# AY-Liu/Image-Editing-Framework

Hardware: AMD Instinct MI355X
Metric: denoising steps/sec (SD1.5 512x512 P2P edit step, UNet batch 4) (higher is better)
Workload: dtype f16x3; 1 GPU; sd15 UNet (859.5M params) P2P AttentionRefine edit step, 2 prompts x CFG = batch 4, 64x64 latents (512x512 px), 50-step DDIM, guidance 7.5, cross 0.8 / self 0.4, per-step null-text unconditional embeddings (P2P_NTI, edit_real.py); one independent edit per GPU; precision mode f16x3: fp32 storage; every contraction on split operands: hi + lo fp16 halves of each fp32 element, Ah Bh + Al Bh + Ah Bl =

## Files before the change

### image-editing-framework_amd/csrc/gemm_x3p.hip

```cpp
#include "ief_common.h"
#include "ief_params.h"
#include "x3_common.h"

#include "x3p_common.h"

template <int BM, int BN, int WAVES_M, int WAVES_N, int NS, int NL, bool CONV>
__global__ __launch_bounds__(64 * (WAVES_M * WAVES_N + NL)) void igemm_x3p_kernel(const IefGemmX3pParams p) {
    constexpr int BK = XP_BK;
    constexpr int NWC = WAVES_M * WAVES_N;
    constexpr int NSW = NL > 0 ? NL : NWC;
    constexpr int PA = BM / 16, PB = BN / 16;
    constexpr int P = 2 * (PA + PB);
    constexpr int G = (P + NSW - 1) / NSW;
    constexpr int WM = BM / WAVES_M, WN = BN / WAVES_N, TM = WM / 16, TN = WN / 16;
    constexpr int SLOT = P * 16 * BK;
    constexpr int DUMP = NS * SLOT;
    static_assert(BM % 16 == 0 && BN % 16 == 0 && WM % 16 == 0 && WN % 16 == 0, "tile");
    static_assert(NS >= 2 && NS <= 4, "ring depth");
    static_assert((NS * SLOT + 512) * 2 <= 160 * 1024, "LDS");
    __shared__ __attribute__((aligned(1024))) half_t smem[NS * SLOT + 512];

    const int tid = threadIdx.x, lane = tid & 63;
    const int wave = __builtin_amdgcn_readfirstlane(tid >> 6);
    const int wr = wave / WAVES_N, wc = wave % WAVES_N;
    const bool stages_ = NL == 0 || wave >= NWC;
    const bool computes = NL == 0 || wave < NWC;
    const int swave = NL > 0 ? wave - NWC : wave;
    const int ntn = (p.N + BN - 1) / BN, ntm = (p.M + BM - 1) / BM;
    const int bid = xcd_remap(blockIdx.x, ntm * ntn);
// ... 23 lines not shown
#pragma unroll
    for (int j = 0; j < G; ++j) {
        const int q = swave + NSW * j;
        exists[j] = stages_ && q < P;
        isA[j] = q < 2 * PA;
        int blk;
        if (isA[j]) { plane[j] = q / PA; blk = q - plane[j] * PA; }
        else { const int q2 = q - 2 * PA; plane[j] = q2 / PB; blk = q2 - plane[j] * PB; }
        ptr[j] = zp; step[j] = 0;
        a_ok[j] = a_live[j] = false; a_y[j] = a_x[j] = a_b[j] = 0; a_m[j] = r1[j] = r2[j] = 0;
        if (!exists[j]) continue;
        if (isA[j]) {
            const int m = m0 + 16 * blk + prow;
            a_ok[j] = m < p.M;
            a_m[j] = (unsigned)m;
            if constexpr (CONV) {
                const int hw = p.Ho * p.Wo;
                const int b = m / hw, rem = m - b * hw;
                const int oy = rem / p.Wo, ox = rem - oy * p.Wo;
                a_b[j] = b;
                a_y[j] = oy * p.stride - (p.pad_hi_only ? 0 : 1);
                a_x[j] = ox * p.stride - (p.pad_hi_only ? 0 : 1);
            } else if (a_ok[j]) {
                ptr[j] = (const char*)p.A + ((long long)plane[j] * p.planeA + (long long)m * p.lda) * 2 + kcb + (long long)kt_lo * (BK * 2);
                step[j] = BK * 2;
            }
        } else {
            const int n = n0 + xp_perm_col<WN>(16 * blk + prow, p.geglu != 0);
            if (n < p.N) {
                ptr[j] = (const char*)p.W + ((long long)plane[j] * p.planeW + (long long)n * p.ldw) * 2 + kcb + (long long)kt_lo * (BK * 2);
                step[j] = BK * 2;
            }
        }
    }

    unsigned stepmask = 0;
#pragma unroll
    for (int j = 0; j < G; ++j) stepmask |= (step[j] != 0 ? 1u : 0u) << j;
    const int Ctot = p.C1 + p.C2;
    const int Hp = p.H >> p.ups, Wp = p.Wd >> p.ups;
    int it_tap = 0, it_c = 0;
    auto set_tap = [&](int tap) {
        if (tap < 9) {
            const int ky = tap / 3, kx = tap - ky * 3;
#pragma unroll
            for (int j = 0; j < G; ++j) {
                if (!(exists[j] && isA[j])) continue;
// ... 8 lines not shown
            for (int j = 0; j < G; ++j) {
                if (!(exists[j] && isA[j])) continue;
                a_live[j] = a_ok[j];
                r1[j] = a_m[j] * (unsigned)p.CE1 * 2u + kcb;
                r2[j] = a_m[j] * (unsigned)p.CE2 * 2u + kcb;
            }
        }
    };
    auto set_src = [&]() {
        const bool tapm = it_tap < 9;
        const int c1 = tapm ? p.C1 : p.CE1;
        const bool first = it_c < c1;
        const char* src = (const char*)(tapm ? (first ? p.A : p.A2) : (first ? p.E1 : p.E2));
        const long long pl = tapm ? (first ? p.planeA : p.planeA2) : (first ? p.planeE1 : p.planeE2);
        const unsigned cc = (unsigned)(first ? it_c : it_c - c1) * 2u;
#pragma unroll
        for (int j = 0; j < G; ++j) {
            if (!(exists[j] && isA[j])) continue;
            ptr[j] = a_live[j] ? src + (long long)plane[j] * pl * 2 + ((first ? r1[j] : r2[j]) + cc) : zp;
            step[j] = a_live[j] ? BK * 2 : 0;
        }
    };

    auto stage_tile = [&](int buf) {
        if (!stages_) return;
        half_t* base = smem + buf * SLOT + swave * (16 * BK);
#pragma unroll
        for (int j = 0; j < G; ++j) {
            half_t* dst = (swave + NSW * j < P) ? base + NSW * j * (16 * BK) : smem + DUMP;
            glds16(ptr[j], dst);
            if constexpr (TN > 5 && !CONV) ptr[j] += ((stepmask >> j) & 1u) ? BK * 2 : 0;
            else ptr[j] += step[j];
        }
        if constexpr (CONV) {
            it_c += BK;
            if (it_tap < 9) {
                if (it_c >= Ctot) { it_c = 0; ++it_tap; set_tap(it_tap); set_src(); }
                else if (it_c == p.C1) set_src();
            } else if (it_c == p.CE1 && p.CE2 > 0) {
                set_src();
            }
        }
    };

    f32x4 acc[TN][TM];
#pragma unroll
    for (int j = 0; j < TN; ++j)
#pragma unroll
        for (int i = 0; i < TM; ++i) acc[j][i] = f32x4{0.f, 0.f, 0.f, 0.f};

    if constexpr (CONV) {
        const int k0 = kt_lo * BK;
        if (k0 < 9 * Ctot) { it_tap = k0 / Ctot; it_c = k0 - it_tap * Ctot; }
        else { it_tap = 9; it_c = k0 - 9 * Ctot; }
        set_tap(it_tap);
// ... 270 lines not shown
    return IEF_OK;
}

extern "C" int ief_gemm_x3p_tile_bm(int tile) {
    switch (tile) {
        case 1: case 2: case 3: case 7: return 128;
        case 4: case 8: case 11: case 12: case 13: return 256;
        case 5: return 64;
        case 6: return 128;
        default: return 0;
    }
}
extern "C" int ief_gemm_x3p_tile_wn(int tile) { return tile == 6 ? 64 : tile == 8 ? 160 : 80; }
extern "C" int ief_gemm_x3p_tile_bn(int tile) {
    switch (tile) {
        case 1: case 2: case 4: case 5: case 7: return 160;
        case 3: case 11: case 12: case 13: return 80;
        case 6: return 64;
        case 8: return 320;
        default: return 0;
    }
}

template <int BM, int BN, int WAVES_M, int WAVES_N, int NS, int NL>
static int launch_x3p(const IefGemmX3pParams& p, hipStream_t st) {
    const int tiles = ((p.M + BM - 1) / BM) * ((p.N + BN - 1) / BN);
    const int splits = p.splits > 1 ? p.splits : 1;
    constexpr int NT = 64 * (WAVES_M * WAVES_N + NL);
    if (p.conv) hipLaunchKernelGGL((igemm_x3p_kernel<BM, BN, WAVES_M, WAVES_N, NS, NL, true>), dim3(tiles, splits), dim3(NT), 0, st, p);
    else hipLaunchKernelGGL((igemm_x3p_kernel<BM, BN, WAVES_M, WAVES_N, NS, NL, false>), dim3(tiles, splits), dim3(NT), 0, st, p);
    IEF_LAUNCH_CHECK();
    return IEF_OK;
}

int ief_conv_halo_x3p_dispatch(const IefGemmX3pParams& p, hipStream_t st);

extern "C" int ief_gemm_x3p(const IefGemmX3pParams* pp, void* stream) {
    if (!pp || !pp->A || !pp->W || !pp->zeros || (!pp->Out && !pp->OutP)) return IEF_EINVAL;
    IefGemmX3pParams p = *pp;
    if (p.M <= 0 || p.N <= 0 || p.K <= 0 || (p.K % XP_BK) || (p.N & 3)) return IEF_ESHAPE;
    if (p.rowvec && p.rows_per_batch <= 0) return IEF_ESHAPE;
    if (p.splits > 1 && (!p.ws || p.splits > 64 || p.geglu || p.rstat_out || p.cstat_out)) return IEF_EINVAL;
    if (!(p.inv_scale > 0.f)) return IEF_EINVAL;
    if ((p.ldw & 7) || (p.planeW & 7) || ((uintptr_t)p.W & 15)) return IEF_EALIGN;
    if (p.Out && ((p.ldo & 3) || ((uintptr_t)p.Out & 15))) return IEF_EALIGN;
    if (p.OutP && ((p.ldp & 3) || (p.planeO & 3) || ((uintptr_t)p.OutP & 7))) return IEF_EALIGN;
    if ((p.bias && ((uintptr_t)p.bias & 15)) || (p.rowvec && ((uintptr_t)p.rowvec & 15)) ||
        (p.residual && (((uintptr_t)p.residual & 15) || (p.ldr & 3)))) return IEF_EALIGN;
    if (p.geglu && ((p.N & 15) || p.residual || p.rowvec)) return IEF_EINVAL;
    if (p.rstat_out && (p.splits > 1 || p.geglu || p.tile == 11 || p.tile == 12 || p.tile == 13 || (p.N % ief_gemm_x3p_tile_wn(p.tile)))) return IEF_EINVAL;
    if (p.rstat_in && (!p.colsum || p.rstat_slots <= 0 || p.rstat_cnt <= 0 || p.rstat_slots * p.rstat_cnt != p.K || p.splits > 1 ||
                       p.conv || !(p.ln_eps > 0.f) || ((uintptr_t)p.colsum & 15))) return IEF_EINVAL;
    if (p.conv) {
        if (p.C1 <= 0 || p.C2 < 0 || (p.C1 % XP_BK) || (p.C2 % XP_BK) || (p.CE1 % XP_BK) || (p.CE2 % XP_BK)) return IEF_ESHAPE;
        if ((p.C2 > 0 && !p.A2) || (p.CE1 > 0 && !p.E1) || (p.CE2 > 0 && !p.E2) || (p.CE2 > 0 && p.CE1 == 0)) return IEF_EINVAL;
        if (p.stride != 1 && p.stride != 2) return IEF_ESHAPE;
        if (p.ups != 0 && p.ups != 1) return IEF_ESHAPE;
        if (p.ups && ((p.H | p.Wd) & 1)) return IEF_ESHAPE;
        if ((p.CE1 + p.CE2) > 0 && (p.stride != 1 || p.ups)) return IEF_ESHAPE;
        const int ktaps = p.tile == 13 ? 4 : 9;
        if (p.K != ktaps * (p.C1 + p.C2) + p.CE1 + p.CE2 || p.batch_images <= 0 || p.M != p.batch_images * p.Ho * p.Wo) return IEF_ESHAPE;
        const long long in_pix = (long long)p.batch_images * (p.H >> p.ups) * (p.Wd >> p.ups);
        const int cmax = p.C1 > p.C2 ? p.C1 : p.C2, emax = p.CE1 > p.CE2 ? p.CE1 : p.CE2;
        if (in_pix * cmax * 2 >= (1ll << 32) || (long long)p.M * emax * 2 >= (1ll << 32)) return IEF_ESHAPE;
        if (((uintptr_t)p.A & 15) || (p.planeA & 7) || (p.A2 && (((uintptr_t)p.A2 & 15) || (p.planeA2 & 7))) ||
            (p.E1 && (((uintptr_t)p.E1 & 15) || (p.planeE1 & 7))) || (p.E2 && (((uintptr_t)p.E2 & 15) || (p.planeE2 & 7)))) return IEF_EALIGN;
    } else {
        if ((p.lda & 7) || (p.planeA & 7) || ((uintptr_t)p.A & 15)) return IEF_EALIGN;
    }
    hipStream_t st = (hipStream_t)stream;
    int rc;
    switch (p.tile) {
        case 2: rc = launch_x3p<128, 160, 4, 2, 4, 4>(p, st); break;
        case 3: rc = launch_x3p<128, 80, 4, 1, 3, 0>(p, st); break;
        case 4: rc = launch_x3p<256, 160, 4, 2, 3, 0>(p, st); break;
        case 5: rc = launch_x3p<64, 160, 2, 2, 4, 0>(p, st); break;
        case 6: rc = launch_x3p<128, 64, 4, 1, 3, 0>(p, st); break;
        case 7: rc = launch_x3p<128, 160, 2, 2, 2, 0>(p, st); break;
        case 8: rc = launch_x3p<256, 320, 4, 2, 2, 0>(p, st); break;
        case 11: case 12: case 13: rc = ief_conv_halo_x3p_dispatch(p, st); break;
        case 1: default: rc = launch_x3p<128, 160, 4, 2, 4, 0>(p, st); break;
    }
    if (rc) return rc;
    if (p.splits > 1) {
        const long long total = (long long)p.M * (p.N / 4);
        int grid = (int)((total + 255) / 256);
        if (grid > 8192) grid = 8192;
        hipLaunchKernelGGL(x3p_reduce_kernel, dim3(grid), dim3(256), 0, st, p);
        IEF_LAUNCH_CHECK();
    }
    return IEF_OK;
}
```

### image-editing-framework_amd/csrc/split_x3.hip

```cpp
#include "ief_common.h"
#include "ief_params.h"

#include "x3_common.h"

__global__ __launch_bounds__(256) void x3_split_weights_kernel(const float* __restrict__ w, half_t* __restrict__ planes, long long n4,
                                                               float s) {
    for (long long i = (long long)blockIdx.x * 256 + threadIdx.x; i < n4; i += (long long)gridDim.x * 256) {
        half4 h, l;
        split4(((const f32x4*)w)[i], s, h, l);
        ((half4*)planes)[i] = h;
        ((half4*)planes)[n4 + i] = l;
    }
}
extern "C" int ief_x3_split_weights(const float* w, void* planes, long long n, float scale, void* stream) {
    if (!w || !planes) return IEF_EINVAL;
    if (n <= 0 || (n & 3) || !(scale > 0.f)) return IEF_ESHAPE;
    if (((uintptr_t)w & 15) || ((uintptr_t)planes & 7)) return IEF_EALIGN;
    long long grid = (n / 4 + 255) / 256;
    if (grid > 16384) grid = 16384;
    hipLaunchKernelGGL(x3_split_weights_kernel, dim3((unsigned)grid), dim3(256), 0, (hipStream_t)stream, w, (half_t*)planes, n / 4, scale);
    IEF_LAUNCH_CHECK();
    return IEF_OK;
}

// ... 8 lines not shown
        const int n = (int)(r % Cout), ph = (int)(r / Cout);
        const int py = ph >> 1, px = ph & 1, sy = tap >> 1, sx = tap & 1;
        const int ky0 = py ? 2 * sy : sy, ky1 = py ? 1 + sy : 2 * sy;
        const int kx0 = px ? 2 * sx : sx, kx1 = px ? 1 + sx : 2 * sx;
        const f32x4* src = (const f32x4*)w + (long long)n * 9 * C4 + c4;
        f32x4 a = src[(ky0 * 3 + kx0) * C4];
        for (int ky = ky0; ky <= ky1; ++ky)
            for (int kx = kx0; kx <= kx1; ++kx)
                if (ky != ky0 || kx != kx0) a = a + src[(ky * 3 + kx) * C4];
        half4 h, l;
        split4(a, s, h, l);
        ((half4*)planes)[i] = h;
        ((half4*)planes)[n4 + i] = l;
    }
}
extern "C" int ief_x3_upsample_phase_weights(const float* w, void* planes, int Cout, int C, float scale, void* stream) {
    if (!w || !planes) return IEF_EINVAL;
    if (Cout <= 0 || C <= 0 || (C & 3) || !(scale > 0.f)) return IEF_ESHAPE;
    if (((uintptr_t)w & 15) || ((uintptr_t)planes & 7)) return IEF_EALIGN;
    long long grid = (16ll * Cout * (C / 4) + 255) / 256;
    if (grid > 16384) grid = 16384;
    hipLaunchKernelGGL(x3_upsample_phase_weights_kernel, dim3((unsigned)grid), dim3(256), 0, (hipStream_t)stream, w, (half_t*)planes, Cout,
                       C / 4, scale);
    IEF_LAUNCH_CHECK();
    return IEF_OK;
}

template <int WM, int WN, int TM, int TN, int KIND, bool TRANSB, bool BPRE>
__global__ __launch_bounds__(64 * WM * WN, (2 * 2 * 16 * (WM * TM + WN * TN) * YLD * 2 > 80 * 1024) ? (WM * WN) / 4 : (WM * WN) / 2)
void igemm_x3_kernel(const IefGemmF32Params p) {
    constexpr bool CONV = KIND >= X3_CONV;
    constexpr bool HASFAST = KIND == X3_LIN || KIND == X3_CONV;
    constexpr int NTH = 64 * WM * WN;
    constexpr int BM = 16 * WM * TM, BN = 16 * WN * TN;
    constexpr int ROWS = BM + BN;
    constexpr int NA = (BM * 8 + NTH - 1) / NTH;
    constexpr int NBC = BPRE ? 2 * BN * 4 : BN * 8;
    constexpr int NB = (NBC + NTH - 1) / NTH;
    constexpr bool A_EXACT = (BM * 8) % NTH == 0, B_EXACT = NBC % NTH == 0;
    static_assert(!(BPRE && TRANSB), "pre-split planes are [N][K]");
    constexpr unsigned OOB = 0xFFFFFFF0u;
    constexpr unsigned OOBF = 0x80000000u;
    __shared__ __attribute__((aligned(16))) half_t smem_y[2 * 2 * ROWS * YLD];
    const int tid = threadIdx.x, lane = tid & 63, wid = tid >> 6;
    const int wm = wid / WN, wn = wid - wm * WN;
    const int lr = lane & 15, lg = lane >> 4;
// ... 1225 lines not shown
```

### image-editing-framework_amd/hip.py

```python
import collections
import ctypes
import os
from ctypes import byref

import torch

from . import cabi

ABI_VERSION = cabi.defines["IEF_ABI_VERSION"]
REPEAT_MAX_JOBS = cabi.defines["IEF_REPEAT_MAX_JOBS"]
_LIB_PATH = os.environ.get("IEF_HIP_LIB") or os.path.join(os.path.dirname(os.path.abspath(__file__)), "libief_hip.so")
_lib = None


class HipExtensionMissing(RuntimeError):
    pass


IefGemmParams = cabi.structs["IefGemmParams"]
IefAttnParams = cabi.structs["IefAttnParams"]
IefCrossParams = cabi.structs["IefCrossParams"]
IefGemmF32Params = cabi.structs["IefGemmF32Params"]
IefAttnF32Params = cabi.structs["IefAttnF32Params"]
IefRepeatJob = cabi.structs["IefRepeatJob"]
# ... 439 lines not shown
    _x3_planes[key] = (weakref.ref(w), w._version, planes)
    weakref.finalize(w, _x3_planes.pop, key, None)
    return planes


def x3_upsample_phase_planes(w, scale=None):
    scale = X3_SCALE_W if scale is None else scale
    key = (w.data_ptr(), tuple(w.shape), float(scale), "phase")
    hit = _x3_planes.get(key)
    if hit is not None and hit[0]() is w and hit[1] == w._version:
        return hit[2]
    if _capturing() or not w.is_contiguous():
        return None
    if w.dim() != 4 or tuple(w.shape[1:3]) != (3, 3) or w.shape[3] % 4:
        raise ValueError("x3_upsample_phase_planes: weight must be [Cout, 3, 3, C] with C a multiple of 4")
    lib = load()
    n, c = w.shape[0], w.shape[3]
    planes = torch.empty(2, 4, n, 4 * c, dtype=torch.float16, device=w.device)
    _check(lib.ief_x3_upsample_phase_weights(w.data_ptr(), planes.data_ptr(), n, c, float(scale), _stream()), "ief_x3_upsample_phase_weights")
    import weakref
    _x3_planes[key] = (weakref.ref(w), w._version, planes)
    weakref.finalize(w, _x3_planes.pop, key, None)
    return planes


def _set_x3(p, sa, sb, w=None) -> str:
    if _F32_CONTRACT == "x3":
        p.x3, p.sa, p.sb = 1, sa, sb
        if w is not None and X3_PRESPLIT and (w.numel() // w.shape[0]) % 8 == 0:
            planes = x3_weight_planes(w, sb)
            if planes is not None:
                p._planes = planes
                p.Wp = planes.data_ptr()
        return "igemm_x3_kernel"
    return "igemm_f32_kernel"


def _is32(t) -> bool:
    return isinstance(t, torch.Tensor) and t.dtype == torch.float32


def _act32(t, name):
    if not (isinstance(t, torch.Tensor) and t.is_cuda and t.dtype == torch.float32):
        raise TypeError(f"{name}: expected an fp32 device tensor (reference-precision mode), got "
                        f"{type(t).__name__ if not isinstance(t, torch.Tensor) else (t.dtype, t.device)}")
    if t.stride(-1) != 1:
# ... 1921 lines not shown
```

### image-editing-framework_amd/planes.py

```python
import os
from ctypes import byref

import torch

from . import hip
from .hip import IefGemmX3pParams, _check, _dev32, _ptr, _shape, _stream, _Timed, _zeros

ACT_SCALE = 1.0
W_SCALE = hip.X3_SCALE_W


class Planes:
    __slots__ = ("t",)

    def __init__(self, t):
        if not (isinstance(t, torch.Tensor) and t.dtype == torch.float16 and t.dim() >= 2 and t.shape[0] == 2 and t.stride(-1) == 1):
            raise TypeError("Planes: expected an fp16 tensor [2, ...] with a contiguous last dimension")
        if not t.is_cuda:
            raise TypeError("Planes: device tensor expected (no CPU path)")
        self.t = t

    @staticmethod
    def empty(*shape, device):
        return Planes(torch.empty(2, *shape, dtype=torch.float16, device=device))
# ... 212 lines not shown
class RowStats:
    __slots__ = ("buf", "slots", "cnt")

    def __init__(self, buf, slots, cnt):
        self.buf, self.slots, self.cnt = buf, slots, cnt


class FoldedLN:
    __slots__ = ("w", "bias", "colsum", "eps")

    def __init__(self, w, bias, gamma, beta, eps):
        wf = (w * gamma[None, :]).contiguous()
        self.w = wf
        b = w @ beta
        self.bias = (b if bias is None else b + bias).contiguous()
        pl = weight_planes(wf)
        self.colsum = ((pl[0].float().sum(1) + pl[1].float().sum(1)) / W_SCALE).contiguous()
        self.eps = eps


LN_FOLD = os.environ.get("IEF_X3P_FOLD_LN", "0") == "1"


def gemm(a, w, bias=None, residual=None, rowvec=None, rows_per_batch=0, out=None, out_planes=None, out_scale=1.0,
         geglu=False, tile=0, splits=0, row_stats=False, ln=None):
    lib = hip.load()
    if not isinstance(a, Planes):
        raise TypeError("planes.gemm: a must be Planes")
    M, K, lda = a.rows_ld("a")
    N = w.shape[0]
    if w.dim() != 2 or w.shape[1] != K:
        raise ValueError(f"planes.gemm: K mismatch {tuple(w.shape)} vs {K}")
    wp = weight_planes(w)
    p = IefGemmX3pParams()
    p.A, p.planeA, p.lda = a.t.data_ptr(), a.plane, lda
    p.W, p.planeW, p.ldw = wp.data_ptr(), wp.stride(0), K
    No = N // 2 if geglu else N
    o32, op = _out_args(p, M, No, out, out_planes, a.device, a.shape[:-1])
    p.M, p.N, p.K = M, N, K
    p.out_scale, p.inv_scale = out_scale, 1.0 / (ACT_SCALE * W_SCALE)
    p.geglu, p.zeros = 1 if geglu else 0, _zeros(a.device)
    if tile:
        p.tile, p.splits = tile, max(1, splits)
    else:
        key = f"gemm|{M}|{N}|{K}" + ("|g" if geglu else "")
        if AUTOTUNE and key not in _plan_table() and not hip._capturing() and hip._prof is None:
            _autotune(key, candidate_plans(M, N, K, geglu=geglu),
                      lambda t, sp, wi: gemm(a, wi, bias=bias, residual=residual, rowvec=rowvec, rows_per_batch=rows_per_batch, out=out,
                                             out_planes=out_planes, out_scale=out_scale, geglu=geglu, tile=t, splits=sp), w)
        p.tile, p.splits = pick_plan(M, N, K, variant="|g" if geglu else "")
    if geglu or row_stats or ln is not None:
        p.splits = 1
    rs = None
    if row_stats:
        wn = lib.ief_gemm_x3p_tile_wn(p.tile)
        if N % wn:
            raise ValueError("planes.gemm: row statistics need N to be a multiple of the tile's wave width")
        rs = RowStats(torch.empty(M, N // wn, 2, dtype=torch.float32, device=a.device), N // wn, wn)
        p.rstat_out = rs.buf.data_ptr()
    if ln is not None:
        st, colsum, eps = ln
        if st.buf.shape[0] != M or st.slots * st.cnt != K or _dev32(colsum, "colsum").numel() != N:
            raise ValueError("planes.gemm: ln statistics / colsum do not match this launch")
        p.rstat_in, p.rstat_slots, p.rstat_cnt, p.colsum, p.ln_eps = st.buf.data_ptr(), st.slots, st.cnt, colsum.data_ptr(), eps
    ws = hip._fill_epilogue(p, hip._rows_ld32, "planes.gemm", M, N, a.device, bias, rowvec, rows_per_batch, residual, p.splits)
    nbytes = 4.0 * (M * K + N * K + M * No * ((1 if o32 is not None else 0) + (1 if op is not None else 0)) + (M * N if residual is not None else 0))
    kn = f"igemm_x3p_kernel<false> t{p.tile}" + (f" {M}x{N}x{K} s{p.splits}" if hip.PROF_SHAPES else "")
    bm, bn = _TILES[p.tile]
    hip.note_staged(kn, 4.0 * K * (bm + bn) * -(-M // bm) * -(-N // bn))
    with _Timed(kn, 2.0 * M * N * K, nbytes):
        _check(lib.ief_gemm_x3p(byref(p), _stream()), "ief_gemm_x3p")
    r = _ret(o32, op)
    if row_stats:
        return (r + (rs,)) if isinstance(r, tuple) else (r, rs)
    return r


def conv3x3(x, w, bias=None, x2=None, stride=1, upsample=False, rowvec=None, residual=None, out=None, out_planes=None,
            extra=None, pad_hi_only=False, tile=0, splits=0):
    lib = hip.load()
    if not isinstance(x, Planes) or (x2 is not None and not isinstance(x2, Planes)):
        raise TypeError("planes.conv3x3: x / x2 must be Planes")
    if not x.is_contiguous() or (x2 is not None and not x2.is_contiguous()) or not w.is_contiguous():
        raise ValueError("planes.conv3x3: x, x2, w must be contiguous")
    e1, e2 = (None, None) if extra is None else extra
    for e in (e1, e2):
        if e is not None and (not isinstance(e, Planes) or not e.is_contiguous()):
            raise ValueError("planes.conv3x3: extra sources must be contiguous NHWC Planes at the output resolution")
    if residual is not None and not hip._act32(residual, "residual").is_contiguous():
        raise ValueError("planes.conv3x3: residual must be contiguous fp32 [B, Ho, Wo, Cout]")
# ... 270 lines not shown
```

### image-editing-framework_amd/unet.py

```python
import math
import os
from typing import Dict, Optional

import torch
from torch import nn

from . import hip, planes
from .config import UNetConfig


FOLD_LN = os.environ.get("IEF_FOLD_LN", "1") == "1"
KV_ONE_GEMM = os.environ.get("IEF_KV_ONE_GEMM", "1") == "1"


def _fold_ln(w16, bias32, gamma, beta):
    wf = w16.float()
    wp = (wf * gamma[None, :]).half().contiguous()
    b = wf @ beta
    if bias32 is not None:
        b = b + bias32
    return wp, b.contiguous(), wp.float().sum(1).contiguous()


class UNetOutput(dict):
# ... 177 lines not shown
                if plan.second_sources(B, self) is not None:
                    raise RuntimeError(f"{self.layer_name}: the Union plan's two key segments exist on the planes attention of the "
                                       "f16x3 mode only")
            o = hip.attn_flash(q, k, v, self.heads, self.scale, q_src=qs, k_src=ks, v_src=vs)
        else:
            q = hip.gemm(x, self.to_q.weight) if ln is None else hip.gemm(x, self.ln_w, bias=self.ln_b, ln=ln)
            kv = self.context_kv(encoder_hidden_states)
            args = plan.cross_edit(B, self) if plan is not None else {}
            if self.map_out is not None:
                hip.attn_probs(q, kv[..., :C], self.heads, self.scale, out=self.map_out)
            o = hip.attn_cross_p2p(q, kv[..., :C], kv[..., C:], self.heads, self.scale, **args)
        if plan is not None:
            plan.layer_done(self)
        lin = self.to_out[0]
        if want_stats:
            return hip.gemm(o, lin.weight, bias=lin.bias, residual=residual, row_stats=True)
        return lin(o, residual=residual)


    def fold_layernorm_x3p(self, norm):
        w = self.w_qkv if self.w_qkv is not None else self.to_q.weight
        self.ln3 = planes.FoldedLN(w, None, norm.weight, norm.bias, norm.eps)

    def forward_x3p(self, xp, ctx, residual, ln_stats=None, want_stats=False, cfg_rows=None):
        B, N, C = xp.shape
        if cfg_rows is not None:
            if cfg_rows.rows != B:
                raise ValueError("forward_x3p: cfg_rows was built for another batch")
            B = cfg_rows.n
        self.last_tokens = N
        plan = self._plan
        w_in, b_in, ln = (self.w_qkv if ctx is None else self.to_q.weight), None, None
        if ln_stats is not None:
            w_in, b_in, ln = self.ln3.w, self.ln3.bias, (ln_stats, self.ln3.colsum, self.ln3.eps)
        if ctx is None:
            qs = ks = vs = None
            if plan is not None:
                qs, ks, vs = plan.self_sources(B, N, self)
            if cfg_rows is not None and (qs is not None or ks is not None or vs is not None
                                         or (plan is not None and plan.mask_launches(B, N, self) is not None)
                                         or (plan is not None and plan.kind == "masactrl_mask_auto"
                                             and (self._exec_index // 2) in plan.masa_layers)):
                raise RuntimeError(f"{self.layer_name}: the control plan acts on a self-attention that runs in the shared prefix of a "
                                   "CFG step (ControlPlan.controls_first_self must say so)")
            if planes.FLASH_PLANES and self.dim_head in planes.FLASH_PLANES_DIMS:
                qkv = planes.gemm(xp, w_in, bias=b_in, ln=ln, out=False, out_planes=True)
                k2 = plan.second_sources(B, self) if plan is not None else None
# ... 18 lines not shown
                qkv = planes.gemm(xp, w_in, bias=b_in, ln=ln)
                if plan is not None and (plan.mask_launches(B, N, self) is not None or plan.auto_launch(B, N, self) is not None):
                    raise RuntimeError(f"mask-guided MasaCtrl was lowered onto a layer of head dim {self.dim_head} that has no "
                                       "planes attention")
                if plan is not None and plan.second_sources(B, self) is not None:
                    raise RuntimeError(f"MasaCtrl Union was lowered onto a layer of head dim {self.dim_head} that has no planes "
                                       "attention")
                o = hip.attn_flash(qkv[..., :C], qkv[..., C:2 * C], qkv[..., 2 * C:], self.heads, self.scale, q_src=qs, k_src=ks,
                                   v_src=vs, out_planes=True)
        else:
            q = planes.gemm(xp, w_in, bias=b_in, ln=ln)
            kv = self.context_kv(ctx)
            args = plan.cross_edit(B, self) if plan is not None else {}
            if self.map_out is not None:
                hip.attn_probs(q, kv[..., :C], self.heads, self.scale, out=self.map_out)
            if plan is not None:
                plan.cross_mass(B, N, self, q, kv[..., :C])
            o = hip.attn_cross_p2p(q, kv[..., :C], kv[..., C:], self.heads, self.scale, out_planes=True, q_src=cfg_rows, **args)
        if plan is not None:
            plan.layer_done(self)
        lin = self.to_out[0]
        if want_stats:
            return planes.gemm(o, lin.weight, bias=lin.bias, residual=residual, out=True, out_planes=True, row_stats=True)
        return planes.gemm(o, lin.weight, bias=lin.bias, residual=residual)


class GEGLU(nn.Module):

    def __init__(self, sd, prefix, dev):
        super().__init__()
        w, b = sd[prefix + ".proj.weight"], sd[prefix + ".proj.bias"]
        half = w.shape[0] // 2
        il = lambda t: torch.stack([t[:half].reshape(half // 8, 8, *t.shape[1:]),
                                    t[half:].reshape(half // 8, 8, *t.shape[1:])], 1).reshape(t.shape)
        self.proj = Linear(_f16(il(w), dev), _f32(il(b), dev))
        self.proj.interleaved = True

    def fold_layernorm(self, norm):
        self.ln_w, self.ln_b, self.ln_c1 = _fold_ln(self.proj.weight, self.proj.bias, norm.weight, norm.bias)
        self.ln_eps = norm.eps

    def forward(self, x, ln_stats=None):
        if ln_stats is not None:
            return hip.gemm(x, self.ln_w, bias=self.ln_b, geglu=True, ln=(ln_stats, self.ln_c1, self.ln_eps))
        return hip.gemm(x, self.proj.weight, bias=self.proj.bias, geglu=True)

# ... 56 lines not shown
        f0 = self.ff.net[0].proj
        self.ff.net[0].ln3 = planes.FoldedLN(f0.weight, f0.bias, self.norm3.weight, self.norm3.bias, self.norm3.eps)

    def foldable_x3p(self):
        if not (planes.LN_FOLD and self.attn1.is_native() and self.attn2.is_native()):
            return False
        if getattr(self.attn1, "ln3", None) is None:
            if hip._capturing():
                return False
            self.fold_layernorm_x3p()
        return True

    def forward_x3p_folded(self, h, hp, st, ctx, last, want_stats):
        h, hp, st = self.attn1.forward_x3p(hp, None, residual=h, ln_stats=st, want_stats=True)
        h, hp, st = self.attn2.forward_x3p(hp, ctx, residual=h, ln_stats=st, want_stats=True)
        f0, lin = self.ff.net[0], self.ff.net[2]
        g = planes.gemm(hp, f0.ln3.w, bias=f0.ln3.bias, geglu=True, out=False, out_planes=True, ln=(st, f0.ln3.colsum, f0.ln3.eps))
        if last:
            return planes.gemm(g, lin.weight, bias=lin.bias, residual=h, out=False, out_planes=True)
        if want_stats:
            return planes.gemm(g, lin.weight, bias=lin.bias, residual=h, out=True, out_planes=True, row_stats=True)
        return planes.gemm(g, lin.weight, bias=lin.bias, residual=h)

    def forward_x3p(self, h, ctx, last, cfg_rows=None, carry=()):
        if cfg_rows is not None:
            h = self.attn1.forward_x3p(planes.layernorm(h, self.norm1.weight, self.norm1.bias, self.norm1.eps), None, residual=h,
                                       cfg_rows=cfg_rows)
            n2 = planes.layernorm(h, self.norm2.weight, self.norm2.bias, self.norm2.eps)
            rep = hip.repeat_batch(h, *carry)
            h, carry = (rep[0], tuple(rep[1:])) if carry else (rep, ())
            h = self.attn2.forward_x3p(n2, ctx, residual=h, cfg_rows=cfg_rows)
        else:
            h = self._attend_x3p(self.attn1, self.norm1, h, None)
            h = self._attend_x3p(self.attn2, self.norm2, h, ctx)
        n3 = planes.layernorm(h, self.norm3.weight, self.norm3.bias, self.norm3.eps)
        f0, lin = self.ff.net[0].proj, self.ff.net[2]
        g = planes.gemm(n3, f0.weight, bias=f0.bias, geglu=True, out=False, out_planes=True)
        if last:
            r = planes.gemm(g, lin.weight, bias=lin.bias, residual=h, out=False, out_planes=True)
        else:
            r = planes.gemm(g, lin.weight, bias=lin.bias, residual=h)
        return (r, carry) if cfg_rows is not None else r


class Transformer2DModel(nn.Module):
    def __init__(self, sd, prefix, dim, heads, cross_dim, groups, dev, name, depth=1):
        super().__init__()
        self.norm = GroupNorm(_f32(sd[prefix + ".norm.weight"], dev), _f32(sd[prefix + ".norm.bias"], dev), groups, 1e-6)
        c1 = lambda n: Conv2d(_f16(sd[f"{prefix}.{n}.weight"].reshape(dim, dim), dev), _f32(sd[f"{prefix}.{n}.bias"], dev), 1)
        self.proj_in, self.proj_out = c1("proj_in"), c1("proj_out")
        self.transformer_blocks = nn.ModuleList(
            [BasicTransformerBlock(sd, f"{prefix}.transformer_blocks.{k}", dim, heads, cross_dim, dev,
                                   name if k == 0 else f"{name}.b{k}") for k in range(depth)])

    def forward(self, x, encoder_hidden_states=None, cstat=None, col_stats=False):
        B, H, W, C = x.shape
        if all(blk.foldable() for blk in self.transformer_blocks):
            h, st = hip.gemm(self.norm(x, cstat=cstat), self.proj_in.weight, bias=self.proj_in.bias, row_stats=True)
            h = h.reshape(B, H * W, C)
            last = len(self.transformer_blocks) - 1
            for k, blk in enumerate(self.transformer_blocks):
                if k < last:
                    h, st = blk(h, encoder_hidden_states, ln_stats=st, want_stats=True)
                else:
                    h = blk(h, encoder_hidden_states, ln_stats=st)
            return self.proj_out(h.reshape(B, H, W, C), residual=x, col_stats=col_stats)
        h = self.proj_in(self.norm(x, cstat=cstat)).reshape(B, H * W, C)
        for blk in self.transformer_blocks:
            h = blk(h, encoder_hidden_states)
        return self.proj_out(h.reshape(B, H, W, C), residual=x, col_stats=col_stats)


    def forward_x3p(self, x, encoder_hidden_states=None, want_planes=False, cfg_rows=None, carry=()):
        B, H, W, C = x.shape
        n = self.norm
        hn = planes.groupnorm(x, n.weight, n.bias, n.num_groups, n.eps, silu=False)
        last = len(self.transformer_blocks) - 1
        if cfg_rows is not None:
            h = planes.gemm(hn.reshape(B, H * W, C), self.proj_in.weight, bias=self.proj_in.bias)
            for k, blk in enumerate(self.transformer_blocks):
                if k == 0:
                    h, rep = blk.forward_x3p(h, encoder_hidden_states, last=(k == last), cfg_rows=cfg_rows, carry=(x,) + tuple(carry))
                    x, carry = rep[0], rep[1:]
                    B = x.shape[0]
                else:
                    h = blk.forward_x3p(h, encoder_hidden_states, last=(k == last))
        elif all(blk.foldable_x3p() for blk in self.transformer_blocks):
            h, hp, st = planes.gemm(hn.reshape(B, H * W, C), self.proj_in.weight, bias=self.proj_in.bias, out=True, out_planes=True,
                                    row_stats=True)
            for k, blk in enumerate(self.transformer_blocks):
                r = blk.forward_x3p_folded(h, hp, st, encoder_hidden_states, last=(k == last), want_stats=(k < last))
                if k < last:
                    h, hp, st = r
                else:
                    h = r
        else:
            h = planes.gemm(hn.reshape(B, H * W, C), self.proj_in.weight, bias=self.proj_in.bias)
            for k, blk in enumerate(self.transformer_blocks):
                h = blk.forward_x3p(h, encoder_hidden_states, last=(k == last))
        r = planes.gemm(h, self.proj_out.weight, bias=self.proj_out.bias, residual=x.reshape(B, H * W, C), out=True,
                        out_planes=want_planes)
        if want_planes:
            r = r[0].reshape(B, H, W, C), r[1].reshape(B, H, W, C)
        else:
            r = r.reshape(B, H, W, C), None
        return r + (tuple(carry),) if cfg_rows is not None else r


class ResnetBlock2D(nn.Module):

    def __init__(self, sd, prefix, cin, cout, groups, eps, dev, temb_slot):
        super().__init__()
        self.in_channels, self.out_channels = cin, cout
        self.norm1 = GroupNorm(_f32(sd[prefix + ".norm1.weight"], dev), _f32(sd[prefix + ".norm1.bias"], dev), groups, eps)
        self.norm2 = GroupNorm(_f32(sd[prefix + ".norm2.weight"], dev), _f32(sd[prefix + ".norm2.bias"], dev), groups, eps)
        pack = lambda w: _f16(w.permute(0, 2, 3, 1), dev)
        self.conv1 = Conv2d(pack(sd[prefix + ".conv1.weight"]), _f32(sd[prefix + ".conv1.bias"], dev), 3)
        self.time_emb_proj = Linear(_f16(sd[prefix + ".time_emb_proj.weight"], dev), _f32(sd[prefix + ".time_emb_proj.bias"], dev))
        self.nonlinearity = SiLU()
        self.dropout = Dropout()
        self.upsample = self.downsample = None
        self.skip_time_act = False
        self.time_embedding_norm = "default"
        self.output_scale_factor = 1.0
# ... 463 lines not shown
```

### include/ief_hip.h

```cpp
#ifndef IEF_HIP_H
#define IEF_HIP_H
#include <stdint.h>

#ifdef __HIPCC__
typedef _Float16 ief_half;
#else
typedef uint16_t ief_half;
#endif

#ifdef __cplusplus
extern "C" {
#endif

#define IEF_ABI_VERSION 4
int ief_abi_version(void);
const char* ief_target_arch(void);
int ief_struct_size(int which);

typedef struct IefGemmParams {
    const ief_half* A;
    const ief_half* A2;
    const ief_half* W;
    ief_half* Out;
    const float* bias;
// ... 224 lines not shown
    const ief_half* W;  long long planeW;
    float* Out;
    ief_half* OutP; long long planeO;
    const float* bias;
    const float* rowvec;
    const float* residual;
    int M, N, K;
    int lda, ldw, ldo, ldp, ldr;
    int conv, H, Wd, C1, C2, Ho, Wo, stride, ups, batch_images, pad_hi_only, CE1, CE2;
    int rows_per_batch;
    float out_scale;
    float inv_scale;
    int tile;
    int splits;
    float* ws;
    int geglu;
    const void* zeros;
    float* rstat_out;
    float* cstat_out;
    const float* rstat_in;
    const float* colsum;
    int rstat_slots, rstat_cnt;
    float ln_eps;
} IefGemmX3pParams;
int ief_gemm_x3p(const IefGemmX3pParams* p, void* stream);
int ief_x3_upsample_phase_weights(const float* w, void* planes, int Cout, int C, float scale, void* stream);
int ief_gemm_x3p_tile_bm(int tile);
int ief_gemm_x3p_tile_bn(int tile);
int ief_gemm_x3p_tile_wn(int tile);
int ief_x3_split_act(const float* x, ief_half* planes, long long plane, long long rows, int C, int ldx, int ldp, float scale,
                     void* stream);

int ief_groupnorm_bwd_f32(const float* x, const float* x2, int C1, int C2, const float* dy, const float* add, float* dx, float* dx2,
                          const float* gamma, const float* beta, int B, int HW, int groups, float eps, int silu, void* stream);
int ief_layernorm_bwd_f32(const float* x, const float* dy, const float* add, float* dx, const float* gamma, long long rows, int C,
                          float eps, void* stream);
int ief_geglu_il_bwd_f32(const float* pre, const float* dy, float* dpre, long long rows, int Ch, void* stream);
int ief_zero_insert2x_f32(const float* in, float* out, int B, int H, int W, int C, void* stream);
int ief_pool2x2_sum_f32(const float* in, float* out, int B, int H, int W, int C, void* stream);
int ief_conv_out_bwd_f32w(const float* d_eps, const float* w, float* dh, int B, int C, int H, int W, int Cout, void* stream);
int ief_softmax_bwd_rows_f32(const float* P, float* dP, long long rows, int L, float scale, void* stream);
int ief_transpose_batched_f32(const float* in, float* out, int R, int N, int L, void* stream);
int ief_map_loss_rows_blocks(long long rows);
int ief_map_loss_rows_f32(const float* P, const float* ref, float* dP, float* loss, long long rows, int L, float gcoef,
                          float loss_coef, void* stream);
int ief_nti_adam_f32g(float* param, float* m, float* v, const float* grad, const float* stats, const float* hyper, int* step, int n,
                      void* stream);

// ... 82 lines not shown
```

### profiles/make_step_breakdown.py

```python
import csv
import json
import sys


def family(n):
    if n.startswith("igemm_x3p_kernel"):
        return "conv (implicit GEMM on planes)" if n.split("(")[0].rstrip(">").endswith("true") else "linear (igemm_x3p)"
    if n.startswith("conv3x3_halo_x3p"):
        return "conv (halo on planes)"
    if n.startswith("attn_flash"):
        return "self-attention (flash)"
    if n.startswith("attn_cross_p2p"):
        return "cross-attention (fused edit)"
    if "gn3_" in n or "groupnorm" in n:
        return "GroupNorm"
    if "layernorm" in n:
        return "LayerNorm"
    if "reduce" in n:
        return "split-K reducer"
    return "other"


def main():
    rows = list(csv.DictReader(open(sys.argv[1])))
    rows.sort(key=lambda r: int(r["Start_Timestamp"]))
    marks = [i for i, r in enumerate(rows) if "cfg_ddim" in r["Kernel_Name"]]
    a, b = marks[len(marks) // 2] + 1, marks[len(marks) // 2 + 1] + 1
    step = rows[a:b]
    out = {"_what": "one captured step of the headline command (f16x3, SD1.5 512x512, batch 4) from profiles' kernel trace: launches and "
                    "kernel time per family", "launches": len(step)}
# ... 20 lines not shown
```

Measured before the change: 80.43 steps/s.

## Fold FF output linear into proj_out via K-concatenated GEMM

```diff
diff --git a/image-editing-framework_amd/csrc/gemm_x3p.hip b/image-editing-framework_amd/csrc/gemm_x3p.hip
--- a/image-editing-framework_amd/csrc/gemm_x3p.hip
+++ b/image-editing-framework_amd/csrc/gemm_x3p.hip
@@ -4,7 +4,7 @@
 
 #include "x3p_common.h"
 
-template <int BM, int BN, int WAVES_M, int WAVES_N, int NS, int NL, bool CONV>
+template <int BM, int BN, int WAVES_M, int WAVES_N, int NS, int NL, bool CONV, bool KCAT = false>
 __global__ __launch_bounds__(64 * (WAVES_M * WAVES_N + NL)) void igemm_x3p_kernel(const IefGemmX3pParams p) {
     constexpr int BK = XP_BK;
     constexpr int NWC = WAVES_M * WAVES_N;
@@ -74,7 +74,14 @@
                 a_y[j] = oy * p.stride - (p.pad_hi_only ? 0 : 1);
                 a_x[j] = ox * p.stride - (p.pad_hi_only ? 0 : 1);
             } else if (a_ok[j]) {
-                ptr[j] = (const char*)p.A + ((long long)plane[j] * p.planeA + (long long)m * p.lda) * 2 + kcb + (long long)kt_lo * (BK * 2);
+                if constexpr (KCAT) {
+                    const int k1t = p.K1 / BK;
+                    ptr[j] = kt_lo < k1t
+                        ? (const char*)p.A + ((long long)plane[j] * p.planeA + (long long)m * p.lda) * 2 + kcb + (long long)kt_lo * (BK * 2)
+                        : (const char*)p.A2 + ((long long)plane[j] * p.planeA2 + (long long)m * p.lda2) * 2 + kcb + (long long)(kt_lo - k1t) * (BK * 2);
+                } else {
+                    ptr[j] = (const char*)p.A + ((long long)plane[j] * p.planeA + (long long)m * p.lda) * 2 + kcb + (long long)kt_lo * (BK * 2);
+                }
                 step[j] = BK * 2;
             }
         } else {
@@ -129,6 +136,7 @@
         }
     };
 
+    int st_k = kt_lo;
     auto stage_tile = [&](int buf) {
         if (!stages_) return;
         half_t* base = smem + buf * SLOT + swave * (16 * BK);
@@ -138,6 +146,14 @@
             glds16(ptr[j], dst);
             if constexpr (TN > 5 && !CONV) ptr[j] += ((stepmask >> j) & 1u) ? BK * 2 : 0;
             else ptr[j] += step[j];
+        }
+        if constexpr (KCAT) {
+            if (++st_k == p.K1 / BK) {
+#pragma unroll
+                for (int j = 0; j < G; ++j)
+                    if (exists[j] && isA[j] && a_ok[j])
+                        ptr[j] = (const char*)p.A2 + ((long long)plane[j] * p.planeA2 + (long long)a_m[j] * p.lda2) * 2 + kcb;
+            }
         }
         if constexpr (CONV) {
             it_c += BK;
@@ -454,13 +470,17 @@
     }
 }
 
-template <int BM, int BN, int WAVES_M, int WAVES_N, int NS, int NL>
+template <int BM, int BN, int WAVES_M, int WAVES_N, int NS, int NL, bool HAS_KCAT = false>
 static int launch_x3p(const IefGemmX3pParams& p, hipStream_t st) {
     const int tiles = ((p.M + BM - 1) / BM) * ((p.N + BN - 1) / BN);
     const int splits = p.splits > 1 ? p.splits : 1;
     constexpr int NT = 64 * (WAVES_M * WAVES_N + NL);
     if (p.conv) hipLaunchKernelGGL((igemm_x3p_kernel<BM, BN, WAVES_M, WAVES_N, NS, NL, true>), dim3(tiles, splits), dim3(NT), 0, st, p);
-    else hipLaunchKernelGGL((igemm_x3p_kernel<BM, BN, WAVES_M, WAVES_N, NS, NL, false>), dim3(tiles, splits), dim3(NT), 0, st, p);
+    else if (p.K1 > 0) {
+        if constexpr (HAS_KCAT)
+            hipLaunchKernelGGL((igemm_x3p_kernel<BM, BN, WAVES_M, WAVES_N, NS, NL, false, true>), dim3(tiles, splits), dim3(NT), 0, st, p);
+        else return IEF_EINVAL;
+    } else hipLaunchKernelGGL((igemm_x3p_kernel<BM, BN, WAVES_M, WAVES_N, NS, NL, false>), dim3(tiles, splits), dim3(NT), 0, st, p);
     IEF_LAUNCH_CHECK();
     return IEF_OK;
 }
@@ -483,6 +503,12 @@
     if (p.rstat_out && (p.splits > 1 || p.geglu || p.tile == 11 || p.tile == 12 || p.tile == 13 || (p.N % ief_gemm_x3p_tile_wn(p.tile)))) return IEF_EINVAL;
     if (p.rstat_in && (!p.colsum || p.rstat_slots <= 0 || p.rstat_cnt <= 0 || p.rstat_slots * p.rstat_cnt != p.K || p.splits > 1 ||
                        p.conv || !(p.ln_eps > 0.f) || ((uintptr_t)p.colsum & 15))) return IEF_EINVAL;
+    if (p.K1 != 0) {
+        if (p.conv || p.geglu || p.rstat_in || !p.A2) return IEF_EINVAL;
+        if (p.tile != 1 && p.tile != 3 && p.tile != 4 && p.tile != 6) return IEF_EINVAL;
+        if (p.K1 < 0 || p.K1 >= p.K || (p.K1 % XP_BK) || ((p.K - p.K1) % XP_BK)) return IEF_ESHAPE;
+        if ((p.lda2 & 7) || (p.planeA2 & 7) || ((uintptr_t)p.A2 & 15)) return IEF_EALIGN;
+    }
     if (p.conv) {
         if (p.C1 <= 0 || p.C2 < 0 || (p.C1 % XP_BK) || (p.C2 % XP_BK) || (p.CE1 % XP_BK) || (p.CE2 % XP_BK)) return IEF_ESHAPE;
         if ((p.C2 > 0 && !p.A2) || (p.CE1 > 0 && !p.E1) || (p.CE2 > 0 && !p.E2) || (p.CE2 > 0 && p.CE1 == 0)) return IEF_EINVAL;
@@ -504,14 +530,14 @@
     int rc;
     switch (p.tile) {
         case 2: rc = launch_x3p<128, 160, 4, 2, 4, 4>(p, st); break;
-        case 3: rc = launch_x3p<128, 80, 4, 1, 3, 0>(p, st); break;
-        case 4: rc = launch_x3p<256, 160, 4, 2, 3, 0>(p, st); break;
+        case 3: rc = launch_x3p<128, 80, 4, 1, 3, 0, true>(p, st); break;
+        case 4: rc = launch_x3p<256, 160, 4, 2, 3, 0, true>(p, st); break;
         case 5: rc = launch_x3p<64, 160, 2, 2, 4, 0>(p, st); break;
-        case 6: rc = launch_x3p<128, 64, 4, 1, 3, 0>(p, st); break;
+        case 6: rc = launch_x3p<128, 64, 4, 1, 3, 0, true>(p, st); break;
         case 7: rc = launch_x3p<128, 160, 2, 2, 2, 0>(p, st); break;
         case 8: rc = launch_x3p<256, 320, 4, 2, 2, 0>(p, st); break;
         case 11: case 12: case 13: rc = ief_conv_halo_x3p_dispatch(p, st); break;
-        case 1: default: rc = launch_x3p<128, 160, 4, 2, 4, 0>(p, st); break;
+        case 1: default: rc = launch_x3p<128, 160, 4, 2, 4, 0, true>(p, st); break;
     }
     if (rc) return rc;
     if (p.splits > 1) {
diff --git a/image-editing-framework_amd/csrc/split_x3.hip b/image-editing-framework_amd/csrc/split_x3.hip
--- a/image-editing-framework_amd/csrc/split_x3.hip
+++ b/image-editing-framework_amd/csrc/split_x3.hip
@@ -54,6 +54,41 @@
     if (grid > 16384) grid = 16384;
     hipLaunchKernelGGL(x3_upsample_phase_weights_kernel, dim3((unsigned)grid), dim3(256), 0, (hipStream_t)stream, w, (half_t*)planes, Cout,
                        C / 4, scale);
+    IEF_LAUNCH_CHECK();
+    return IEF_OK;
+}
+
+__global__ __launch_bounds__(256) void x3_fold_linear_pair_kernel(const float* __restrict__ wp, const float* __restrict__ w2,
+                                                                  const float* __restrict__ b2, const float* __restrict__ bp,
+                                                                  float* __restrict__ wcat, float* __restrict__ bcat, int C, int K) {
+    const int cols = K + C + 1;
+    const long long total = (long long)C * cols;
+    for (long long i = (long long)blockIdx.x * 256 + threadIdx.x; i < total; i += (long long)gridDim.x * 256) {
+        const int r = (int)(i / cols), c = (int)(i - (long long)r * cols);
+        const float* wr = wp + (long long)r * C;
+        if (c < K) {
+            double a = 0.0;
+            for (int j = 0; j < C; ++j) a += (double)wr[j] * (double)w2[(long long)j * K + c];
+            wcat[(long long)r * (K + C) + c] = (float)a;
+        } else if (c < K + C) {
+            wcat[(long long)r * (K + C) + c] = wr[c - K];
+        } else {
+            double a = 0.0;
+            if (b2)
+                for (int j = 0; j < C; ++j) a += (double)wr[j] * (double)b2[j];
+            if (bp) a += (double)bp[r];
+            bcat[r] = (float)a;
+        }
+    }
+}
+extern "C" int ief_x3_fold_linear_pair(const float* wp, const float* w2, const float* b2, const float* bp, float* wcat, float* bcat,
+                                       int C, int K, void* stream) {
+    if (!wp || !w2 || !wcat || !bcat) return IEF_EINVAL;
+    if (C <= 0 || K <= 0) return IEF_ESHAPE;
+    long long grid = ((long long)C * (K + C + 1) + 255) / 256;
+    if (grid > 16384) grid = 16384;
+    hipLaunchKernelGGL(x3_fold_linear_pair_kernel, dim3((unsigned)grid), dim3(256), 0, (hipStream_t)stream, wp, w2, b2, bp, wcat, bcat, C,
+                       K);
     IEF_LAUNCH_CHECK();
     return IEF_OK;
 }
diff --git a/image-editing-framework_amd/hip.py b/image-editing-framework_amd/hip.py
--- a/image-editing-framework_amd/hip.py
+++ b/image-editing-framework_amd/hip.py
@@ -485,6 +485,44 @@
     _x3_planes[key] = (weakref.ref(w), w._version, planes)
     weakref.finalize(w, _x3_planes.pop, key, None)
     return planes
+
+
+def fold_linear_pair_ref(wp, w2, b2=None, bp=None):
+    wp64, w264 = wp.double(), w2.double()
+    if wp64.dim() != 2 or wp64.shape[0] != wp64.shape[1] or w264.dim() != 2 or w264.shape[0] != wp64.shape[0]:
+        raise ValueError("fold_linear_pair: wp must be [C, C] and w2 [C, K]")
+    b = torch.zeros(wp64.shape[0], dtype=torch.float64, device=wp.device)
+    if b2 is not None:
+        b = wp64 @ b2.double()
+    if bp is not None:
+        b = b + bp.double()
+    return torch.cat([wp64 @ w264, wp64], 1), b
+
+
+def x3_fold_linear_pair(wp, w2, b2=None, bp=None):
+    key = (wp.data_ptr(), tuple(wp.shape), w2.data_ptr(), tuple(w2.shape), "fold")
+    srcs = (wp, w2, b2, bp)
+    hit = _x3_planes.get(key)
+    if hit is not None and all((r is None and t is None) or (r is not None and r() is t and v == t._version)
+                               for t, (r, v) in zip(srcs, hit[0])):
+        return hit[2]
+    if _capturing():
+        return None
+    if wp.dim() != 2 or wp.shape[0] != wp.shape[1] or w2.dim() != 2 or w2.shape[0] != wp.shape[0]:
+        raise ValueError("x3_fold_linear_pair: wp must be [C, C] and w2 [C, K]")
+    C, K = w2.shape
+    for t, nm in ((wp, "wp"), (w2, "w2"), (b2, "b2"), (bp, "bp")):
+        if t is not None and (not _dev32(t, nm).is_contiguous() or (t.dim() == 1 and t.numel() != C)):
+            raise ValueError(f"x3_fold_linear_pair: {nm} must be contiguous fp32 ([C] for a bias)")
+    lib = load()
+    wcat = torch.empty(C, K + C, dtype=torch.float32, device=wp.device)
+    bcat = torch.empty(C, dtype=torch.float32, device=wp.device)
+    _check(lib.ief_x3_fold_linear_pair(wp.data_ptr(), w2.data_ptr(), _ptr(b2), _ptr(bp), wcat.data_ptr(), bcat.data_ptr(), C, K,
+                                       _stream()), "ief_x3_fold_linear_pair")
+    import weakref
+    _x3_planes[key] = (tuple((None, 0) if t is None else (weakref.ref(t), t._version) for t in srcs), 0, (wcat, bcat))
+    weakref.finalize(wp, _x3_planes.pop, key, None)
+    return wcat, bcat
 
 
 def _set_x3(p, sa, sb, w=None) -> str:
diff --git a/image-editing-framework_amd/planes.py b/image-editing-framework_amd/planes.py
--- a/image-editing-framework_amd/planes.py
+++ b/image-editing-framework_amd/planes.py
@@ -258,18 +258,37 @@
 LN_FOLD = os.environ.get("IEF_X3P_FOLD_LN", "0") == "1"
 
 
+KCAT_TILES = (1, 3, 4, 6)
+_KCAT_NEAREST = {2: 1, 5: 1, 7: 1, 8: 4}
+
+
+FOLD_TAIL = os.environ.get("IEF_X3P_FOLD_TAIL", "1") == "1"
+
+
 def gemm(a, w, bias=None, residual=None, rowvec=None, rows_per_batch=0, out=None, out_planes=None, out_scale=1.0,
-         geglu=False, tile=0, splits=0, row_stats=False, ln=None):
+         geglu=False, tile=0, splits=0, row_stats=False, ln=None, a2=None):
     lib = hip.load()
     if not isinstance(a, Planes):
         raise TypeError("planes.gemm: a must be Planes")
     M, K, lda = a.rows_ld("a")
+    K1 = 0
+    if a2 is not None:
+        if not isinstance(a2, Planes):
+            raise TypeError("planes.gemm: a2 must be Planes")
+        if geglu or ln is not None:
+            raise ValueError("planes.gemm: a K-concatenated launch takes no geglu and no folded LayerNorm")
+        M2, K2, lda2 = a2.rows_ld("a2")
+        if M2 != M:
+            raise ValueError(f"planes.gemm: a2 has {M2} rows, a has {M}")
+        K1, K = K, K + K2
     N = w.shape[0]
     if w.dim() != 2 or w.shape[1] != K:
         raise ValueError(f"planes.gemm: K mismatch {tuple(w.shape)} vs {K}")
     wp = weight_planes(w)
     p = IefGemmX3pParams()
     p.A, p.planeA, p.lda = a.t.data_ptr(), a.plane, lda
+    if a2 is not None:
+        p.A2, p.planeA2, p.lda2, p.K1 = a2.t.data_ptr(), a2.plane, lda2, K1
     p.W, p.planeW, p.ldw = wp.data_ptr(), wp.stride(0), K
     No = N // 2 if geglu else N
     o32, op = _out_args(p, M, No, out, out_planes, a.device, a.shape[:-1])
@@ -281,10 +300,13 @@
     else:
         key = f"gemm|{M}|{N}|{K}" + ("|g" if geglu else "")
         if AUTOTUNE and key not in _plan_table() and not hip._capturing() and hip._prof is None:
-            _autotune(key, candidate_plans(M, N, K, geglu=geglu),
+            cands = candidate_plans(M, N, K, geglu=geglu)
+            _autotune(key, [c for c in cands if a2 is None or c[0] in KCAT_TILES],
                       lambda t, sp, wi: gemm(a, wi, bias=bias, residual=residual, rowvec=rowvec, rows_per_batch=rows_per_batch, out=out,
-                                             out_planes=out_planes, out_scale=out_scale, geglu=geglu, tile=t, splits=sp), w)
+                                             out_planes=out_planes, out_scale=out_scale, geglu=geglu, tile=t, splits=sp, a2=a2), w)
         p.tile, p.splits = pick_plan(M, N, K, variant="|g" if geglu else "")
+        if a2 is not None:
+            p.tile = _KCAT_NEAREST.get(p.tile, p.tile)
     if geglu or row_stats or ln is not None:
         p.splits = 1
     rs = None
@@ -301,7 +323,7 @@
         p.rstat_in, p.rstat_slots, p.rstat_cnt, p.colsum, p.ln_eps = st.buf.data_ptr(), st.slots, st.cnt, colsum.data_ptr(), eps
     ws = hip._fill_epilogue(p, hip._rows_ld32, "planes.gemm", M, N, a.device, bias, rowvec, rows_per_batch, residual, p.splits)
     nbytes = 4.0 * (M * K + N * K + M * No * ((1 if o32 is not None else 0) + (1 if op is not None else 0)) + (M * N if residual is not None else 0))
-    kn = f"igemm_x3p_kernel<false> t{p.tile}" + (f" {M}x{N}x{K} s{p.splits}" if hip.PROF_SHAPES else "")
+    kn = f"igemm_x3p_kernel<false>{' kcat' if a2 is not None else ''} t{p.tile}" + (f" {M}x{N}x{K} s{p.splits}" if hip.PROF_SHAPES else "")
     bm, bn = _TILES[p.tile]
     hip.note_staged(kn, 4.0 * K * (bm + bn) * -(-M // bm) * -(-N // bn))
     with _Timed(kn, 2.0 * M * N * K, nbytes):
diff --git a/image-editing-framework_amd/unet.py b/image-editing-framework_amd/unet.py
--- a/image-editing-framework_amd/unet.py
+++ b/image-editing-framework_amd/unet.py
@@ -223,7 +223,7 @@
         w = self.w_qkv if self.w_qkv is not None else self.to_q.weight
         self.ln3 = planes.FoldedLN(w, None, norm.weight, norm.bias, norm.eps)
 
-    def forward_x3p(self, xp, ctx, residual, ln_stats=None, want_stats=False, cfg_rows=None):
+    def forward_x3p(self, xp, ctx, residual, ln_stats=None, want_stats=False, cfg_rows=None, want_planes=False):
         B, N, C = xp.shape
         if cfg_rows is not None:
             if cfg_rows.rows != B:
@@ -288,6 +288,8 @@
         lin = self.to_out[0]
         if want_stats:
             return planes.gemm(o, lin.weight, bias=lin.bias, residual=residual, out=True, out_planes=True, row_stats=True)
+        if want_planes:
+            return planes.gemm(o, lin.weight, bias=lin.bias, residual=residual, out=True, out_planes=True)
         return planes.gemm(o, lin.weight, bias=lin.bias, residual=residual)
 
 
@@ -390,21 +392,30 @@
             return planes.gemm(g, lin.weight, bias=lin.bias, residual=h, out=True, out_planes=True, row_stats=True)
         return planes.gemm(g, lin.weight, bias=lin.bias, residual=h)
 
-    def forward_x3p(self, h, ctx, last, cfg_rows=None, carry=()):
+    def forward_x3p(self, h, ctx, last, cfg_rows=None, carry=(), fold_tail=False):
         if cfg_rows is not None:
             h = self.attn1.forward_x3p(planes.layernorm(h, self.norm1.weight, self.norm1.bias, self.norm1.eps), None, residual=h,
                                        cfg_rows=cfg_rows)
             n2 = planes.layernorm(h, self.norm2.weight, self.norm2.bias, self.norm2.eps)
             rep = hip.repeat_batch(h, *carry)
             h, carry = (rep[0], tuple(rep[1:])) if carry else (rep, ())
-            h = self.attn2.forward_x3p(n2, ctx, residual=h, cfg_rows=cfg_rows)
+            h = self.attn2.forward_x3p(n2, ctx, residual=h, cfg_rows=cfg_rows, want_planes=fold_tail)
         else:
             h = self._attend_x3p(self.attn1, self.norm1, h, None)
-            h = self._attend_x3p(self.attn2, self.norm2, h, ctx)
+            if fold_tail:
+                h = self.attn2.forward_x3p(planes.layernorm(h, self.norm2.weight, self.norm2.bias, self.norm2.eps), ctx, residual=h,
+                                           want_planes=True)
+            else:
+                h = self._attend_x3p(self.attn2, self.norm2, h, ctx)
+        hp = None
+        if fold_tail:
+            h, hp = h
         n3 = planes.layernorm(h, self.norm3.weight, self.norm3.bias, self.norm3.eps)
         f0, lin = self.ff.net[0].proj, self.ff.net[2]
         g = planes.gemm(n3, f0.weight, bias=f0.bias, geglu=True, out=False, out_planes=True)
-        if last:
+        if fold_tail:
+            r = (g, hp)
+        elif last:
             r = planes.gemm(g, lin.weight, bias=lin.bias, residual=h, out=False, out_planes=True)
         else:
             r = planes.gemm(g, lin.weight, bias=lin.bias, residual=h)
@@ -439,20 +450,30 @@
         return self.proj_out(h.reshape(B, H, W, C), residual=x, col_stats=col_stats)
 
 
+    def tail_fold(self):
+        blk = self.transformer_blocks[-1]
+        if not planes.FOLD_TAIL or planes.LN_FOLD or not blk.attn2.is_native():
+            return None
+        lin = blk.ff.net[2]
+        return hip.x3_fold_linear_pair(self.proj_out.weight, lin.weight, lin.bias, self.proj_out.bias)
+
     def forward_x3p(self, x, encoder_hidden_states=None, want_planes=False, cfg_rows=None, carry=()):
         B, H, W, C = x.shape
         n = self.norm
         hn = planes.groupnorm(x, n.weight, n.bias, n.num_groups, n.eps, silu=False)
         last = len(self.transformer_blocks) - 1
+        fold = self.tail_fold()
         if cfg_rows is not None:
             h = planes.gemm(hn.reshape(B, H * W, C), self.proj_in.weight, bias=self.proj_in.bias)
             for k, blk in enumerate(self.transformer_blocks):
+                ft = fold is not None and k == last
                 if k == 0:
-                    h, rep = blk.forward_x3p(h, encoder_hidden_states, last=(k == last), cfg_rows=cfg_rows, carry=(x,) + tuple(carry))
+                    h, rep = blk.forward_x3p(h, encoder_hidden_states, last=(k == last), cfg_rows=cfg_rows, carry=(x,) + tuple(carry),
+                                             fold_tail=ft)
                     x, carry = rep[0], rep[1:]
                     B = x.shape[0]
                 else:
-                    h = blk.forward_x3p(h, encoder_hidden_states, last=(k == last))
+                    h = blk.forward_x3p(h, encoder_hidden_states, last=(k == last), fold_tail=ft)
         elif all(blk.foldable_x3p() for blk in self.transformer_blocks):
             h, hp, st = planes.gemm(hn.reshape(B, H * W, C), self.proj_in.weight, bias=self.proj_in.bias, out=True, out_planes=True,
                                     row_stats=True)
@@ -465,9 +486,13 @@
         else:
             h = planes.gemm(hn.reshape(B, H * W, C), self.proj_in.weight, bias=self.proj_in.bias)
             for k, blk in enumerate(self.transformer_blocks):
-                h = blk.forward_x3p(h, encoder_hidden_states, last=(k == last))
-        r = planes.gemm(h, self.proj_out.weight, bias=self.proj_out.bias, residual=x.reshape(B, H * W, C), out=True,
-                        out_planes=want_planes)
+                h = blk.forward_x3p(h, encoder_hidden_states, last=(k == last), fold_tail=(fold is not None and k == last))
+        if fold is not None:
+            g, hp = h
+            r = planes.gemm(g, fold[0], a2=hp, bias=fold[1], residual=x.reshape(B, H * W, C), out=True, out_planes=want_planes)
+        else:
+            r = planes.gemm(h, self.proj_out.weight, bias=self.proj_out.bias, residual=x.reshape(B, H * W, C), out=True,
+                            out_planes=want_planes)
         if want_planes:
             r = r[0].reshape(B, H, W, C), r[1].reshape(B, H, W, C)
         else:
diff --git a/include/ief_hip.h b/include/ief_hip.h
--- a/include/ief_hip.h
+++ b/include/ief_hip.h
@@ -270,8 +270,11 @@
     const float* colsum;
     int rstat_slots, rstat_cnt;
     float ln_eps;
+    int K1, lda2;
 } IefGemmX3pParams;
 int ief_gemm_x3p(const IefGemmX3pParams* p, void* stream);
+int ief_x3_fold_linear_pair(const float* wp, const float* w2, const float* b2, const float* bp, float* wcat, float* bcat, int C, int K,
+                            void* stream);
 int ief_x3_upsample_phase_weights(const float* w, void* planes, int Cout, int C, float scale, void* stream);
 int ief_gemm_x3p_tile_bm(int tile);
 int ief_gemm_x3p_tile_bn(int tile);
diff --git a/profiles/make_step_breakdown.py b/profiles/make_step_breakdown.py
--- a/profiles/make_step_breakdown.py
+++ b/profiles/make_step_breakdown.py
@@ -5,7 +5,8 @@
 
 def family(n):
     if n.startswith("igemm_x3p_kernel"):
-        return "conv (implicit GEMM on planes)" if n.split("(")[0].rstrip(">").endswith("true") else "linear (igemm_x3p)"
+        args = n.split("(")[0].split("<", 1)[1].rstrip(">").split(", ")
+        return "conv (implicit GEMM on planes)" if args[6] == "true" else "linear (igemm_x3p)"
     if n.startswith("conv3x3_halo_x3p"):
         return "conv (halo on planes)"
     if n.startswith("attn_flash"):
```

After: 81.85 steps/s, median of 6. 1.02x the previous value.
